# connortannahill/MM-ADMM

Hardware: AMD Instinct MI355X
Metric: ADMM iterations/sec on 1M-node 2D mesh; achieved HBM GB/s in SpMV (higher is better)
Workload: dtype f64

## Files before the change

mm-admm_amd/csrc/host/engine.cpp:

```cpp
#include <algorithm>
#include <chrono>
#include <cmath>
#include <cstring>
#include <limits>
#include <memory>
#include <mutex>
#include <string>
#include <vector>

#include "../../../include/mmx_sparse.h"
#include "../kernels/admm_kernels.h"
#include "../kernels/field_kernels.h"
#include "../kernels/quality_kernels.h"
#include "../kernels/regrid_kernels.h"
#include "../kernels/transfer_kernels.h"
#include "comm.h"
#include "common.h"
#include "partition.h"
#include "transfer.h"
#include "xup_records.h"

#define MMX_SP(expr)                                                                     \
  do {                                                                                   \
    const int rc_ = (expr);                                                              \
// ... 1172 lines not shown
    const CellGrid cg = cellGrid(lo, hi);
    int marg[3] = {0, 0, 0};
    const GridBox R = rowBox(llo, lhi, marg);
    const int passes = smoothPasses();
    const GridBox H = widenBox(R, passes);
    double slo[3] = {0, 0, 0}, shi[3] = {0, 0, 0};
    double diam = 0.0;
    for (int d = 0; d < D; ++d) diam += extMax_[d] * extMax_[d];
    diam = std::sqrt(diam);
    const double marginScale = knobs_.regridMargin;
    for (int d = 0; d < D; ++d) {
      const std::vector<double>& g = d == 0 ? grid_.gx : d == 1 ? grid_.gy : grid_.gz;
      const int sd = (D == 3 && d < 2) ? 1 - d : d;
      const double mu = marginScale * (diam + 2.0 * (g[1] - g[0]));
      slo[d] = g[H.lo[sd]] - mu;
      shi[d] = g[H.hi[sd]] + mu;
    }
    for (int d = 0; d < D; ++d) {
      hs[d] = slo[d];
      hs[D + d] = shi[d];
    }
    smallGather(hs, 2 * D);
    MMX_HIP(hipMemcpyAsync(rgnSbox_.p, hr, sizeof(double) * nranks_ * 2 * D, hipMemcpyHostToDevice, st_));
    MMX_HIP(hipMemsetAsync(rgnCnt_.p, 0, sizeof(int) * (nranks_ + 1), st_));
    launch_select_owned<D>(Vp_.p, ownLocal_.p, rgnOwnGid_.p, nOwned_, nranks_, rank_, rgnSbox_.p, rgnCnt_.p,
                           rgnSend_.p, maxOwned_, st_);
    std::vector<int> cnt(nranks_ + 1);
    MMX_HIP(hipMemcpyAsync(cnt.data(), rgnCnt_.p, sizeof(int) * nranks_, hipMemcpyDeviceToHost, st_));
    streamWait();
    for (int q = 0; q < nranks_; ++q) hs[q] = (double)cnt[q];
    smallGather(hs, nranks_);
    std::vector<HaloPeer> peers;
    int nRecv = 0;
    for (int q = 0; q < nranks_; ++q) {
      if (q == rank_) continue;
      const int sc = cnt[q], rc = (int)hr[(size_t)q * nranks_ + rank_];
      if (sc == 0 && rc == 0) continue;
      HaloPeer p;
      p.rank = q;
      p.sendOff = q * maxOwned_;
      p.sendCount = sc;
      p.recvOff = nRecv;
      p.recvCount = rc;
      nRecv += rc;
      peers.push_back(p);
    }
    const int nCand = nP_ + nRecv;
    if ((int)rgnRecv_.n < std::max(nRecv, 1) * (D + 1)) rgnRecv_.alloc((size_t)std::max(nRecv, 1) * (D + 1) * 2);
    if ((int)rgnCandX_.n < nCand * D) {
      rgnCandX_.alloc((size_t)nCand * D * 2);
      rgnCandGid_.alloc((size_t)nCand * 2);
      rgnCellOf_.alloc((size_t)nCand * 2);
      rgnNodes_.alloc((size_t)nCand * 2);
      rgnMon_.alloc((size_t)nCand * DD * 2);
    }
    comm_->exchange(rank_, rgnSend_.p, rgnRecv_.p, peers, D + 1, st_);
    launch_build_cand<D>(Vp_.p, rgnGid_.p, nP_, rgnRecv_.p, nRecv, rgnCandX_.p, rgnCandGid_.p, st_);
    evalMonitorAt(rgnCandX_.p, nCand, t, rgnMon_.p);
    ensureCells(cg);
    launch_bin<D>(rgnCandX_.p, nCand, cg, rgnCellOf_.p, rgCounts_.p, rgStarts_.p, rgFill_.p, rgnNodes_.p, rgScan_.p,
                  rgScanBytes_, st_);
    double clo[3], chi[3];
    for (int d = 0; d < 3; ++d) {
      clo[d] = (d < D && slo[d] <= lo[d]) ? -INFINITY : slo[d];
      chi[d] = (d < D && shi[d] >= hi[d]) ? INFINITY : shi[d];
    }
    NnCand nc{rgnCandGid_.p, {clo[0], clo[1], clo[2]}, {chi[0], chi[1], chi[2]}, rgnCnt_.p + nranks_};
    launch_nn_fill<D>(rgnCandX_.p, cg, rgStarts_.p, rgnNodes_.p, gx_.p, gy_.p, D == 3 ? gz_.p : gy_.p, grid_.nx,
                      grid_.ny, grid_.nz, rgnMon_.p, rgTmp_.p, H, st_, nc);
    int fail = 0;
    MMX_HIP(hipMemcpyAsync(&fail, rgnCnt_.p + nranks_, sizeof(int), hipMemcpyDeviceToHost, st_));
    streamWait();
    hs[0] = (double)fail;
    smallGather(hs, 1);
    for (int q = 0; q < nranks_; ++q)
      if (hr[q] != 0.0) return false;
    smoothCommit(R, passes, true);
    st_stats_.regrid_rows = (long long)(H.hi[0] - H.lo[0] + 1) * (H.hi[1] - H.lo[1] + 1) * (H.hi[2] - H.lo[2] + 1);
    st_stats_.regrid_gather_bytes = (double)sizeof(double) * ((size_t)nranks_ * (4 * D + nranks_ + 1) +
                                                              (size_t)nRecv * (D + 1));
    st_stats_.regrid_cand = nCand;
    MMX_HIP(hipGetLastError());
    gridOnDevice_ = true;
    updateIso();
    m_ = makeView();
    st_stats_.regrids += 1;
    return true;
  }

  void updateIso() {
    iso_ = false;
    if (!knobs_.iso) return;
    const long long np = (long long)(gvals_.n / (D * D));
    if (np <= 0) return;
    if ((long long)giso_.n != np) giso_.alloc(np);
    if (!isoFlag_.p) isoFlag_.alloc(1);
    MMX_HIP(hipMemsetAsync(isoFlag_.p, 0, sizeof(int), st_));
    launch_iso_compact<D>(gvals_.p, np, giso_.p, isoFlag_.p, st_);
    int notIso = 1;
    MMX_HIP(hipMemcpyAsync(&notIso, isoFlag_.p, sizeof(int), hipMemcpyDeviceToHost, st_));
    streamWait();
    iso_ = (notIso == 0);
  }
  void uploadGridCoords() {
    gx_.upload(grid_.gx.data(), grid_.gx.size(), st_);
    gy_.upload(grid_.gy.data(), grid_.gy.size(), st_);
    if (D == 3) {
      gz_.upload(grid_.gz.data(), grid_.gz.size(), st_);
      const std::vector<double>* ax[3] = {&grid_.gx, &grid_.gy, &grid_.gz};
      for (int a = 0; a < 3; ++a) {
        const std::vector<double>& g = *ax[a];
        const size_t nc = g.size() > 1 ? g.size() - 1 : 1;
        std::vector<double>& t = gcellH_[a];
        t.assign(4 * nc, 0.0);
        for (size_t i = 0; i + 1 < g.size(); ++i) {
          const double h = g[i + 1] - g[i];
          t[4 * i] = g[i];
          t[4 * i + 1] = h;
          t[4 * i + 2] = 1.0 / h;
        }
        gcell_[a].upload(t.data(), t.size(), st_);
      }
    }
  }
  void setGridGeometry(int nG, const double* lo, const double* hi) {
    grid_geometry(D, nG, lo, hi, grid_);
    uploadGridCoords();
  }
  CellGrid cellGrid(const double* lo, const double* hi) const {
    CellGrid cg{};
    const int gn[3] = {grid_.nx, grid_.ny, grid_.nz};
    cg.hmin = INFINITY;
    for (int d = 0; d < 3; ++d) {
      const double ext = d < D ? hi[d] - lo[d] : 0.0;
      cg.lo[d] = d < D ? lo[d] : 0.0;
      cg.n[d] = (d < D && ext > 0) ? std::max(1, gn[d] / 2) : 1;
      cg.inv[d] = (d < D && ext > 0) ? cg.n[d] / ext : 0.0;
      if (d < D && ext > 0) cg.hmin = std::min(cg.hmin, ext / cg.n[d]);
    }
    if (!(cg.hmin < INFINITY)) cg.hmin = 0.0;
    return cg;
  }
  void ensureCells(const CellGrid& cg) {
    const int ncell = cg.n[0] * cg.n[1] * cg.n[2];
    if ((int)rgStarts_.n < ncell + 1) {
      rgCounts_.alloc(ncell + 1);
      rgStarts_.alloc(ncell + 1);
      rgFill_.alloc(ncell);
      rgScanBytes_ = bin_scan_bytes(ncell);
      rgScan_.alloc(std::max<size_t>(rgScanBytes_, 1));
    }
  }
  static int smoothPasses() { return (D == 2) ? 5 : 2; }
  GridBox rowBox(const double* llo, const double* lhi, int* marg) const {
    const int gn3[3] = {grid_.nx, grid_.ny, D == 3 ? grid_.nz : 0};
    GridBox R{{0, 0, 0}, {gn3[0], gn3[1], gn3[2]}};
    for (int d = 0; d < D; ++d) {
      const std::vector<double>& g = d == 0 ? grid_.gx : d == 1 ? grid_.gy : grid_.gz;
      const double h = g[1] - g[0];
      const int M = (int)std::ceil(2.0 * extMax_[d] / h) + 2;
      marg[d] = M;
      R.lo[d] = std::max(0, std::min(gn3[d], (int)std::floor((llo[d] - g[0]) / h) - M));
      R.hi[d] = std::max(0, std::min(gn3[d], (int)std::floor((lhi[d] - g[0]) / h) + 1 + M));
    }
    return R;
  }
  GridBox widenBox(const GridBox& b, int w) const {
    const int gn3[3] = {grid_.nx, grid_.ny, D == 3 ? grid_.nz : 0};
    GridBox o = b;
    for (int d = 0; d < D; ++d) {
      o.lo[d] = std::max(0, b.lo[d] - w);
      o.hi[d] = std::min(gn3[d], b.hi[d] + w);
    }
    return o;
  }
  void evalMonitorAt(const double* X, int n, double t, double* mon) {
    constexpr int DD = D * D;
    if (builtin_monitor_kind(monFn_, monUser_) == 7) {
      double c[3];
      moving_bump_centre(t, c);
      launch_monitor_tv<D>(X, n, c, mon, st_);
    } else {
      std::vector<double> Xh((size_t)n * D), mv((size_t)n * DD);
      MMX_HIP(hipMemcpyAsync(Xh.data(), X, Xh.size() * sizeof(double), hipMemcpyDeviceToHost, st_));
      streamWait();
      for (int v = 0; v < n; ++v) {
        double M[9];
        for (int i = 0; i < DD; ++i) M[i] = 0.0;
        monFn_(D, &Xh[(size_t)v * D], M, monUser_);
        std::memcpy(&mv[(size_t)v * DD], M, DD * sizeof(double));
      }
      MMX_HIP(hipMemcpyAsync(mon, mv.data(), mv.size() * sizeof(double), hipMemcpyHostToDevice, st_));
      streamWait();
    }
  }
  void smoothCommit(const GridBox& R, int passes, bool part) {
    double* cur = rgTmp_.p;
    double* oth = part ? rgTmp2_.p : gvals_.p;
    for (int it = 0; it < passes; ++it) {
      launch_smooth<D>(cur, oth, grid_.nx, grid_.ny, grid_.nz, widenBox(R, part ? passes - 1 - it : 0), st_);
      std::swap(cur, oth);
    }
    if (part) {
      launch_box_commit<D>(cur, gvals_.p, D == 3 ? gpad_.p : nullptr, grid_.nx, grid_.ny, grid_.nz, R, st_);
    } else {
      if (cur != gvals_.p)
        MMX_HIP(hipMemcpyAsync(gvals_.p, cur, gvals_.n * sizeof(double), hipMemcpyDeviceToDevice, st_));
      if (D == 3) launch_pad_rows(gvals_.p, (long long)(gvals_.n / 9), gpad_.p, st_);
    }
  }

  void regridAll(double t, MonSource src = kMonCallback) {
    constexpr int DD = D * D;
    const int nG = (nranks_ > 1) ? plan_.nP : nP_;
    const int nb = std::max(1, std::min(256, (nG + 255) / 256));
    if (!rgPart_.p) {
      rgPart_.alloc((size_t)512 * 2 * D + 256 * D);
      rgMon_.alloc((size_t)nG * DD);
      rgCellOf_.alloc(nG);
      rgNodes_.alloc(nG);
      rgTmp_.alloc(gvals_.n);
      if (nranks_ > 1) rgTmp2_.alloc(gvals_.n);
      if (nranks_ > 1) {
        rgXg_.alloc((size_t)nG * D);
        rgSend_.alloc((size_t)maxOwned_ * D);
        rgRecv_.alloc((size_t)nranks_ * maxOwned_ * D);
      }
      MMX_HIP(hipHostMalloc((void**)&rgHost_, sizeof(double) * (512 * 2 * D + 256 * D), hipHostMallocDefault));
    }
    const double* X = Vp_.p;
    const bool part = nranks_ > 1;
    const int nbl = part ? std::max(1, std::min(256, (nP_ + 255) / 256)) : 0;
    const int nbe = part ? std::max(1, std::min(256, (nF_ + 255) / 256)) : 0;
    double* extPart = rgPart_.p + (size_t)512 * 2 * D;
    if (part) {
      launch_rows_gather(D, ownLocal_.p, nOwned_, Vp_.p, rgSend_.p, st_);
      comm_->allgather(rank_, rgSend_.p, rgRecv_.p, (size_t)maxOwned_ * D, st_);
      launch_rows_scatter(D, ownAllGid_.p, nranks_ * maxOwned_, rgRecv_.p, rgXg_.p, st_);
      X = rgXg_.p;
      launch_bbox<D>(Vp_.p, nP_, rgPart_.p + (size_t)256 * 2 * D, nbl, st_);
      launch_extent<D>(Vp_.p, F_.p, nF_, extPart, nbe, st_);
    }
    launch_bbox<D>(X, nG, rgPart_.p, nb, st_);
    MMX_HIP(hipMemcpyAsync(rgHost_, rgPart_.p, sizeof(double) * nb * 2 * D, hipMemcpyDeviceToHost, st_));
    if (part) {
      MMX_HIP(hipMemcpyAsync(rgHost_ + (size_t)256 * 2 * D, rgPart_.p + (size_t)256 * 2 * D, sizeof(double) * nbl * 2 * D,
                             hipMemcpyDeviceToHost, st_));
      MMX_HIP(hipMemcpyAsync(rgHost_ + (size_t)512 * 2 * D, extPart, sizeof(double) * nbe * D, hipMemcpyDeviceToHost,
                             st_));
    }
    streamWait();
    double lo[3] = {INFINITY, INFINITY, INFINITY}, hi[3] = {-INFINITY, -INFINITY, -INFINITY};
    double llo[3] = {INFINITY, INFINITY, INFINITY}, lhi[3] = {-INFINITY, -INFINITY, -INFINITY};
    for (int b = 0; b < nb; ++b)
      for (int d = 0; d < D; ++d) {
        lo[d] = std::min(lo[d], rgHost_[(size_t)b * 2 * D + d]);
        hi[d] = std::max(hi[d], rgHost_[(size_t)b * 2 * D + D + d]);
      }
    for (int b = 0; b < nbl; ++b)
      for (int d = 0; d < D; ++d) {
        llo[d] = std::min(llo[d], rgHost_[(size_t)(256 + b) * 2 * D + d]);
        lhi[d] = std::max(lhi[d], rgHost_[(size_t)(256 + b) * 2 * D + D + d]);
      }
    if (part) {
      for (int d = 0; d < D; ++d) extMax_[d] = 0.0;
      for (int b = 0; b < nbe; ++b)
        for (int d = 0; d < D; ++d) extMax_[d] = std::max(extMax_[d], rgHost_[(size_t)512 * 2 * D + (size_t)b * D + d]);
    }
    grid_geometry(D, nG, lo, hi, grid_);
    uploadGridCoords();
    CellGrid cg{};
    const int gn[3] = {grid_.nx, grid_.ny, grid_.nz};
    cg.hmin = INFINITY;
    for (int d = 0; d < 3; ++d) {
      const double ext = d < D ? hi[d] - lo[d] : 0.0;
      cg.lo[d] = d < D ? lo[d] : 0.0;
      cg.n[d] = (d < D && ext > 0) ? std::max(1, gn[d] / 2) : 1;
      cg.inv[d] = (d < D && ext > 0) ? cg.n[d] / ext : 0.0;
      if (d < D && ext > 0) cg.hmin = std::min(cg.hmin, ext / cg.n[d]);
    }
    if (!(cg.hmin < INFINITY)) cg.hmin = 0.0;
    const int ncell = cg.n[0] * cg.n[1] * cg.n[2];
    if ((int)rgStarts_.n < ncell + 1) {
      rgCounts_.alloc(ncell + 1);
      rgStarts_.alloc(ncell + 1);
      rgFill_.alloc(ncell);
      rgScanBytes_ = bin_scan_bytes(ncell);
      rgScan_.alloc(std::max<size_t>(rgScanBytes_, 1));
    }
    launch_bin<D>(X, nG, cg, rgCellOf_.p, rgCounts_.p, rgStarts_.p, rgFill_.p, rgNodes_.p, rgScan_.p, rgScanBytes_,
                  st_);
    if (src == kMonCallback && builtin_monitor_kind(monFn_, monUser_) == 7) src = kMonBuiltin7;
    if (src == kMonValues) {
      MMX_HIP(hipMemcpyAsync(rgMon_.p, srcPtr_, (size_t)nG * DD * sizeof(double), hipMemcpyDeviceToDevice, st_));
    } else if (src == kMonField) {
      fieldScratch();
      launch_field_hessian<D>(X, srcPtr_, F_.p, nF_, incPtr_.p, incOff_.p, nodeOrder_.p, nP_, fldE_.p, fldG_.p,
                              srcAlpha_, nullptr, rgMon_.p, st_);
    } else if (src == kMonFieldHuang) {
      fieldHuangMonitor(X);
    } else if (src == kMonBuiltin7) {
      double c[3];
      moving_bump_centre(t, c);
      launch_monitor_tv<D>(X, nG, c, rgMon_.p, st_);
    } else {
      std::vector<double> Xh((size_t)nG * D), mv((size_t)nG * DD);
      MMX_HIP(hipMemcpyAsync(Xh.data(), X, Xh.size() * sizeof(double), hipMemcpyDeviceToHost, st_));
      streamWait();
      for (int v = 0; v < nG; ++v) {
        double M[9];
        for (int i = 0; i < DD; ++i) M[i] = 0.0;
        monFn_(D, &Xh[(size_t)v * D], M, monUser_);
        std::memcpy(&mv[(size_t)v * DD], M, DD * sizeof(double));
      }
      MMX_HIP(hipMemcpyAsync(rgMon_.p, mv.data(), mv.size() * sizeof(double), hipMemcpyHostToDevice, st_));
      streamWait();
    }
    const int passes = (D == 2) ? 5 : 2;
    const int gn3[3] = {grid_.nx, grid_.ny, D == 3 ? grid_.nz : 0};
    GridBox R{{0, 0, 0}, {gn3[0], gn3[1], gn3[2]}};
    if (part) {
      for (int d = 0; d < D; ++d) {
        const std::vector<double>& g = d == 0 ? grid_.gx : d == 1 ? grid_.gy : grid_.gz;
        const double h = g[1] - g[0];
        const int M = (int)std::ceil(2.0 * extMax_[d] / h) + 2;
        R.lo[d] = std::max(0, std::min(gn3[d], (int)std::floor((llo[d] - g[0]) / h) - M));
        R.hi[d] = std::max(0, std::min(gn3[d], (int)std::floor((lhi[d] - g[0]) / h) + 1 + M));
      }
    }
    auto widen = [&](const GridBox& b, int w) {
      GridBox o = b;
      for (int d = 0; d < D; ++d) {
        o.lo[d] = std::max(0, b.lo[d] - w);
        o.hi[d] = std::min(gn3[d], b.hi[d] + w);
      }
      return o;
    };
    const GridBox H = widen(R, part ? passes : 0);
    launch_nn_fill<D>(X, cg, rgStarts_.p, rgNodes_.p, gx_.p, gy_.p, D == 3 ? gz_.p : gy_.p, grid_.nx, grid_.ny,
                      grid_.nz, rgMon_.p, rgTmp_.p, H, st_);
    double* cur = rgTmp_.p;
    double* oth = part ? rgTmp2_.p : gvals_.p;
    for (int it = 0; it < passes; ++it) {
      launch_smooth<D>(cur, oth, grid_.nx, grid_.ny, grid_.nz, widen(R, part ? passes - 1 - it : 0), st_);
      std::swap(cur, oth);
    }
    if (part) {
      launch_box_commit<D>(cur, gvals_.p, D == 3 ? gpad_.p : nullptr, grid_.nx, grid_.ny, grid_.nz, R, st_);
    } else {
      if (cur != gvals_.p)
        MMX_HIP(hipMemcpyAsync(gvals_.p, cur, gvals_.n * sizeof(double), hipMemcpyDeviceToDevice, st_));
      if (D == 3) launch_pad_rows(gvals_.p, (long long)(gvals_.n / 9), gpad_.p, st_);
    }
    st_stats_.regrid_rows = (long long)(H.hi[0] - H.lo[0] + 1) * (H.hi[1] - H.lo[1] + 1) * (H.hi[2] - H.lo[2] + 1);
    st_stats_.regrid_gather_bytes = part ? (double)nranks_ * maxOwned_ * D * sizeof(double) : 0.0;
    st_stats_.regrid_cand = part ? nG : 0;
    MMX_HIP(hipGetLastError());
    gridOnDevice_ = true;
    updateIso();
    m_ = makeView();
    st_stats_.regrids += 1;
  }

  DeviceMesh<D> makeView() const {
    DeviceMesh<D> m{};
    m.nP = nP_;
    m.nF = nF_;
    m.F = F_.p;
    m.sbits = sbits_.p;
    m.nodeInterior = interior_.p;
    m.inc_ptr = incPtr_.p;
    m.inc_off = incOff_.p;
    m.remote = nranks_ > 1 ? remote_.p : nullptr;
    m.tslot = knobs_.tslot ? tslot_.p : nullptr;
    m.gcache = gcache_.p;
    m.tieList = tieList_.p;
    m.tieCount = tieCount_.p + tiePar_;
    m.tieStale = tieCount_.p + (tiePar_ ^ 1);
    m.invFlag = tieCount_.p + 2;
    m.nodeOrder = nodeOrder_.p;
    m.xupLo = 0;
    m.xupHi = nP_;
    m.prox2dWave = knobs_.prox2dWave;
    m.xupSweep = knobs_.xupSweep;
    m.xupCh = knobs_.xupCh;
    m.xupEarly = knobs_.xupEarly;
    m.forceTie = knobs_.forceTie;
    m.monHint = knobs_.monHint;
    if (knobs_.xupRec) {
      m.xrec = xrec_.p;
      m.xinv = xinv_.p;
      m.xslot = xslot_.p;
      m.xslotStride = xslotStride_;
      m.xslotCh = xslotCh_;
    }
    m.invdiag = invdiag_.p;
    m.Vc = compMesh_ ? Vc_.p : nullptr;
    m.gx = gx_.p;
    m.gy = gy_.p;
    m.gz = (D == 3) ? gz_.p : gy_.p;
    m.gvals = gvals_.p;
    m.gpad = (D == 3) ? gpad_.p : nullptr;
    for (int a = 0; a < 3; ++a) m.gcell[a] = (D == 3) ? gcell_[a].p : nullptr;
    m.giso = iso_ ? giso_.p : nullptr;
    m.gnx = grid_.nx;
    m.gny = grid_.ny;
    m.gnz = grid_.nz;
    m.ghx = grid_.gx[1] - grid_.gx[0];
    m.ghy = grid_.gy[1] - grid_.gy[0];
    m.ghz = (D == 3) ? grid_.gz[1] - grid_.gz[0] : 1.0;
    m.grhx = 1.0 / m.ghx;
    m.grhy = 1.0 / m.ghy;
    m.grhz = 1.0 / m.ghz;
    const int ns[3] = {grid_.nx, grid_.ny, grid_.nz};
    double* A[3] = {&m.gax, &m.gay, &m.gaz};
    double* SP[3] = {&m.gspx, &m.gspy, &m.gspz};
    double* NS[3] = {&m.gnsx, &m.gnsy, &m.gnsz};
    double* RNS[3] = {&m.grnsx, &m.grnsy, &m.grnsz};
    for (int d = 0; d < 3; ++d) {
      const bool on = d < D;
      *A[d] = on ? grid_.lo[d] : 0.0;
      *SP[d] = on ? grid_.hi[d] - grid_.lo[d] : 0.0;
      *NS[d] = on ? (double)ns[d] : 1.0;
      *RNS[d] = 1.0 / *NS[d];
    }
    for (int i = 0; i < D * D; ++i) m.Ehat[i] = EhatH_[i];
    m.powd = powd_;
    m.w = w_;
    m.compMesh = compMesh_ ? 1 : 0;
    return m;
  }

  void ensureResults(int nIters) {
    if (nIters <= resultsCap_) return;
    resultsCap_ = std::max(nIters, 64);
    const size_t n = (size_t)resultsCap_ * 2 * kNumPartials;
    if (nranks_ == 1 && knobs_.spin) {
      if (resH_) MMX_HIP(hipHostFree(resH_));
      resH_ = nullptr;
      MMX_HIP(hipHostMalloc((void**)&resH_, n * sizeof(double), hipHostMallocMapped));
      MMX_HIP(hipHostGetDevicePointer((void**)&res_, resH_, 0));
    } else {
// ... 452 lines not shown
```

mm-admm_amd/csrc/kernels/regrid_kernels.h:

```cpp
#pragma once
#include <hip/hip_runtime.h>
#include <stddef.h>

namespace mmx {

struct CellGrid {
  double lo[3];
  double inv[3];
  int n[3];
  double hmin;
};

struct GridBox {
  int lo[3];
  int hi[3];
};

template <int D>
void launch_bbox(const double* X, int n, double* partials, int nblocks, hipStream_t st);
template <int D>
void launch_extent(const double* X, const int* F, int nF, double* partials, int nblocks, hipStream_t st);
template <int D>
void launch_bin(const double* X, int n, const CellGrid& cg, int* cellOfV, int* counts, int* starts, int* fill,
                int* cellNodes, void* scanTmp, size_t scanTmpBytes, hipStream_t st);
size_t bin_scan_bytes(int ncell);
template <int D>
void launch_monitor_tv(const double* X, int n, const double* c, double* monVals, hipStream_t st);
struct NnCand {
  const int* gid;
  double slo[3], shi[3];
  int* fail;
};
template <int D>
void launch_nn_fill(const double* X, const CellGrid& cg, const int* starts, const int* cellNodes, const double* gx,
                    const double* gy, const double* gz, int nx, int ny, int nz, const double* monVals, double* vals,
                    const GridBox& box, hipStream_t st, const NnCand& cand = NnCand{nullptr, {0, 0, 0}, {0, 0, 0}, nullptr});
template <int D>
void launch_select_owned(const double* X, const int* ownLocal, const int* ownGid, int nOwned, int nranks, int rank,
                         const double* sboxes, int* counts, double* send, int cap, hipStream_t st);
template <int D>
void launch_build_cand(const double* X, const int* gidLocal, int nLocal, const double* recv, int nRecv, double* cx,
                       int* cgid, hipStream_t st);
template <int D>
void launch_smooth(const double* in, double* out, int nx, int ny, int nz, const GridBox& box, hipStream_t st);
template <int D>
void launch_box_commit(const double* src, double* vals, double* pad, int nx, int ny, int nz, const GridBox& box,
                       hipStream_t st);

void launch_rows_gather(int D, const int* idx, int n, const double* in, double* out, hipStream_t st);
void launch_rows_scatter(int D, const int* idx, int n, const double* in, double* out, hipStream_t st);

}
```

mm-admm_amd/csrc/kernels/regrid_kernels.hip:

```cpp
#include <hip/hip_runtime.h>

#include <hipcub/hipcub.hpp>

#include "regrid_kernels.h"

namespace mmx {
namespace {

constexpr int kRB = 256;

template <int D>
__global__ void __launch_bounds__(kRB) k_bbox(const double* __restrict__ X, int n, double* __restrict__ part) {
  __shared__ double sm[2 * D][kRB];
  double lo[D], hi[D];
#pragma unroll
  for (int d = 0; d < D; ++d) {
    lo[d] = INFINITY;
    hi[d] = -INFINITY;
  }
  for (int v = blockIdx.x * kRB + threadIdx.x; v < n; v += gridDim.x * kRB)
#pragma unroll
    for (int d = 0; d < D; ++d) {
      const double x = X[(size_t)v * D + d];
      lo[d] = x < lo[d] ? x : lo[d];
// ... 30 lines not shown
#pragma unroll
    for (int n = 0; n <= D; ++n) v[n] = F[(size_t)s * (D + 1) + n];
#pragma unroll
    for (int d = 0; d < D; ++d) {
      double a = X[(size_t)v[0] * D + d], b = a;
#pragma unroll
      for (int n = 1; n <= D; ++n) {
        const double c = X[(size_t)v[n] * D + d];
        a = c < a ? c : a;
        b = c > b ? c : b;
      }
      const double e = b - a;
      ext[d] = e > ext[d] ? e : ext[d];
    }
  }
#pragma unroll
  for (int d = 0; d < D; ++d) sm[d][threadIdx.x] = ext[d];
  __syncthreads();
  for (int w = kRB / 2; w > 0; w >>= 1) {
    if ((int)threadIdx.x < w)
#pragma unroll
      for (int d = 0; d < D; ++d) {
        const double a = sm[d][threadIdx.x + w];
        sm[d][threadIdx.x] = a > sm[d][threadIdx.x] ? a : sm[d][threadIdx.x];
      }
    __syncthreads();
  }
  if (threadIdx.x < D) part[(size_t)blockIdx.x * D + threadIdx.x] = sm[threadIdx.x][0];
}

template <int D>
__device__ __forceinline__ int cellOf(const double* x, const CellGrid& cg, int (&c)[3]) {
  int id = 0;
#pragma unroll
  for (int d = D - 1; d >= 0; --d) {
    int k = (int)((x[d] - cg.lo[d]) * cg.inv[d]);
    k = k < 0 ? 0 : (k >= cg.n[d] ? cg.n[d] - 1 : k);
    c[d] = k;
    id = id * cg.n[d] + k;
  }
  return id;
}

template <int D>
__global__ void __launch_bounds__(kRB) k_bin_count(const double* __restrict__ X, int n, CellGrid cg,
                                                   int* __restrict__ cellOfV, int* __restrict__ counts) {
  const int v = blockIdx.x * kRB + threadIdx.x;
  if (v >= n) return;
  double x[D];
#pragma unroll
  for (int d = 0; d < D; ++d) x[d] = X[(size_t)v * D + d];
  int c[3];
  const int id = cellOf<D>(x, cg, c);
  cellOfV[v] = id;
  atomicAdd(&counts[id], 1);
}

__global__ void __launch_bounds__(kRB) k_bin_fill(int n, const int* __restrict__ cellOfV,
                                                  const int* __restrict__ starts, int* __restrict__ fill,
                                                  int* __restrict__ cellNodes) {
  const int v = blockIdx.x * kRB + threadIdx.x;
  if (v >= n) return;
  const int c = cellOfV[v];
  cellNodes[starts[c] + atomicAdd(&fill[c], 1)] = v;
}

template <int D>
__global__ void __launch_bounds__(kRB) k_monitor_tv(const double* __restrict__ X, int n, double c0, double c1,
                                                    double c2, double* __restrict__ monVals) {
  const int v = blockIdx.x * kRB + threadIdx.x;
  if (v >= n) return;
  const double c[3] = {c0, c1, c2};
  double sq = 0.0;
#pragma unroll
  for (int d = 0; d < D; ++d) {
    const double t = X[(size_t)v * D + d] - c[d];
    sq = (d == 0) ? t * t : sq + t * t;
  }
  const double s = 1 + 5.0 / (1 + 50.0 * sq);
#pragma unroll
  for (int i = 0; i < D * D; ++i) monVals[(size_t)v * D * D + i] = (i / D == i % D) ? s : 0.0;
}

__device__ __forceinline__ size_t box_row(const GridBox& b, long long p, int nx, int ny, int& sx, int& sy, int& sk) {
  const long long bx = b.hi[0] - b.lo[0] + 1, by = b.hi[1] - b.lo[1] + 1;
  sx = b.lo[0] + (int)(p % bx);
  sy = b.lo[1] + (int)((p / bx) % by);
  sk = b.lo[2] + (int)(p / (bx * by));
  return ((size_t)sk * (ny + 1) + sy) * (nx + 1) + sx;
}
__device__ __forceinline__ long long box_rows(const GridBox& b) {
  return (long long)(b.hi[0] - b.lo[0] + 1) * (b.hi[1] - b.lo[1] + 1) * (b.hi[2] - b.lo[2] + 1);
}

template <int D>
__global__ void __launch_bounds__(kRB) k_nn_fill(const double* __restrict__ X, CellGrid cg,
                                                 const int* __restrict__ starts, const int* __restrict__ cellNodes,
                                                 const double* __restrict__ gx, const double* __restrict__ gy,
                                                 const double* __restrict__ gz, int nx, int ny, int nz,
                                                 const double* __restrict__ monVals, double* __restrict__ vals,
                                                 GridBox box, NnCand cand) {
  constexpr int DD = D * D;
  const long long p = (long long)blockIdx.x * kRB + threadIdx.x;
  if (p >= box_rows(box)) return;
  int sx, sy, k;
  const size_t row = box_row(box, p, nx, ny, sx, sy, k);
  const int i = (D == 2) ? sx : sy, j = (D == 2) ? sy : sx;
  double q[3] = {gx[i], gy[j], D == 3 ? gz[k] : 0.0};
  int c[3] = {0, 0, 0};
  cellOf<D>(q, cg, c);
  double best = INFINITY;
  int bi = -1, bg = -1;
  int rmax = 0;
#pragma unroll
  for (int d = 0; d < D; ++d) rmax = max(rmax, max(c[d], cg.n[d] - 1 - c[d]));
  for (int r = 0; r <= rmax; ++r) {
    const int z0 = (D == 3) ? max(c[2] - r, 0) : 0, z1 = (D == 3) ? min(c[2] + r, cg.n[2] - 1) : 0;
    const int y0 = max(c[1] - r, 0), y1 = min(c[1] + r, cg.n[1] - 1);
    const int x0 = max(c[0] - r, 0), x1 = min(c[0] + r, cg.n[0] - 1);
    for (int cz = z0; cz <= z1; ++cz)
      for (int cy = y0; cy <= y1; ++cy)
        for (int cx = x0; cx <= x1; ++cx) {
          const int dz = (D == 3) ? abs(cz - c[2]) : 0;
          if (max(max(abs(cx - c[0]), abs(cy - c[1])), dz) != r) continue;
          const int cell = (cz * cg.n[1] + cy) * cg.n[0] + cx;
          for (int t = starts[cell]; t < starts[cell + 1]; ++t) {
            const int v = cellNodes[t];
            const int gv = cand.gid ? cand.gid[v] : v;
            double dd = 0.0;
#pragma unroll
            for (int d = 0; d < D; ++d) {
              const double df = q[d] - X[(size_t)v * D + d];
              dd += df * df;
            }
            if (dd < best || (dd == best && gv < bg)) {
              best = dd;
              bi = v;
              bg = gv;
            }
          }
        }
    const double lb = ((double)r - 1e-6) * cg.hmin;
    if (bi >= 0 && r > 0 && best < lb * lb) break;
  }
  if (cand.gid) {
    double gap = INFINITY;
#pragma unroll
    for (int d = 0; d < D; ++d) gap = fmin(gap, fmin(q[d] - cand.slo[d], cand.shi[d] - q[d]));
    if (!(bi >= 0 && gap > 0.0 && best < gap * gap * (1.0 - 1e-9))) {
      atomicOr(cand.fail, 1);
      if (bi < 0) return;
    }
  }
#pragma unroll
  for (int e = 0; e < DD; ++e) vals[row * DD + e] = monVals[(size_t)bi * DD + e];
}

template <int D>
__global__ void __launch_bounds__(kRB) k_select_owned(const double* __restrict__ X, const int* __restrict__ ownLocal,
                                                      const int* __restrict__ ownGid, int nOwned, int nranks, int rank,
                                                      const double* __restrict__ sboxes, int* __restrict__ counts,
                                                      double* __restrict__ send, int cap) {
  const int i = blockIdx.x * kRB + threadIdx.x;
  if (i >= nOwned) return;
  const int v = ownLocal[i];
  double x[D];
#pragma unroll
  for (int d = 0; d < D; ++d) x[d] = X[(size_t)v * D + d];
  for (int q = 0; q < nranks; ++q) {
    if (q == rank) continue;
    const double* s = sboxes + (size_t)q * 2 * D;
    bool in = true;
#pragma unroll
    for (int d = 0; d < D; ++d) in = in && x[d] >= s[d] && x[d] <= s[D + d];
    if (in) {
      const int k = atomicAdd(&counts[q], 1);
      double* r = send + ((size_t)q * cap + k) * (D + 1);
#pragma unroll
      for (int d = 0; d < D; ++d) r[d] = x[d];
      r[D] = (double)ownGid[i];
    }
  }
}

template <int D>
__global__ void __launch_bounds__(kRB) k_build_cand(const double* __restrict__ X, const int* __restrict__ gidLocal,
                                                    int nLocal, const double* __restrict__ recv, int nRecv,
                                                    double* __restrict__ cx, int* __restrict__ cgid) {
  const int i = blockIdx.x * kRB + threadIdx.x;
  if (i >= nLocal + nRecv) return;
  if (i < nLocal) {
#pragma unroll
    for (int d = 0; d < D; ++d) cx[(size_t)i * D + d] = X[(size_t)i * D + d];
    cgid[i] = gidLocal[i];
  } else {
    const double* r = recv + (size_t)(i - nLocal) * (D + 1);
#pragma unroll
    for (int d = 0; d < D; ++d) cx[(size_t)i * D + d] = r[d];
    cgid[i] = (int)r[D];
  }
}

template <int D>
__global__ void __launch_bounds__(kRB) k_smooth(const double* __restrict__ in, double* __restrict__ out, int nx,
                                                int ny, int nz, GridBox box) {
  constexpr int DD = D * D;
  const long long p = (long long)blockIdx.x * kRB + threadIdx.x;
  const long long P = (long long)(nx + 1) * (ny + 1);
  if (p >= box_rows(box)) return;
  int i, j, k;
  const long long c = (long long)box_row(box, p, nx, ny, i, j, k);
  const bool interior = i >= 1 && i < nx && j >= 1 && j < ny && (D == 2 || (k >= 1 && k < nz));
  for (int q = 0; q < DD; ++q) {
    double v;
    if (!interior) {
      v = in[c * DD + q];
    } else if constexpr (D == 2) {
      v = 0.6 * in[c * DD + q];
      v += 0.1 * in[(c + 1) * DD + q];
      v += 0.1 * in[(c - 1) * DD + q];
      v += 0.1 * in[(c + nx + 1) * DD + q];
      v += 0.1 * in[(c - nx - 1) * DD + q];
    } else {
      const double h = 0.4 / 6.0;
      v = 0.6 * in[c * DD + q] + h * in[(c + 1) * DD + q] + h * in[(c - 1) * DD + q] + h * in[(c + nx + 1) * DD + q] +
          h * in[(c - nx - 1) * DD + q] + h * in[(c + P) * DD + q] + h * in[(c - P) * DD + q];
    }
    out[c * DD + q] = v;
  }
}

template <int D>
__global__ void __launch_bounds__(kRB) k_box_commit(const double* __restrict__ src, double* __restrict__ vals,
                                                    double* __restrict__ pad, int nx, int ny, int nz, GridBox box) {
  constexpr int DD = D * D;
  const long long c = (long long)blockIdx.x * kRB + threadIdx.x;
  const long long P = (long long)(nx + 1) * (ny + 1);
  if (c >= P * (D == 3 ? nz + 1 : 1)) return;
  const int i = (int)(c % (nx + 1)), j = (int)((c / (nx + 1)) % (ny + 1)), k = (D == 3) ? (int)(c / P) : 0;
  const bool in = i >= box.lo[0] && i <= box.hi[0] && j >= box.lo[1] && j <= box.hi[1] && k >= box.lo[2] &&
                  k <= box.hi[2];
  const double nan = __builtin_nan("");
  for (int q = 0; q < DD; ++q) vals[c * DD + q] = in ? src[c * DD + q] : nan;
  if (D == 3 && pad) {
    for (int q = 0; q < DD; ++q) pad[c * 10 + q] = in ? src[c * DD + q] : nan;
    pad[c * 10 + 9] = 0.0;
  }
}

__global__ void __launch_bounds__(kRB) k_rows_gather(int D, const int* __restrict__ idx, int n,
                                                     const double* __restrict__ in, double* __restrict__ out) {
  const int i = blockIdx.x * kRB + threadIdx.x;
  if (i >= n) return;
  for (int c = 0; c < D; ++c) out[(size_t)i * D + c] = in[(size_t)idx[i] * D + c];
}
__global__ void __launch_bounds__(kRB) k_rows_scatter(int D, const int* __restrict__ idx, int n,
                                                      const double* __restrict__ in, double* __restrict__ out) {
  const int i = blockIdx.x * kRB + threadIdx.x;
  if (i >= n || idx[i] < 0) return;
  for (int c = 0; c < D; ++c) out[(size_t)idx[i] * D + c] = in[(size_t)i * D + c];
}

inline unsigned blocks(long long n) { return (unsigned)((n + kRB - 1) / kRB); }

}

template <int D>
void launch_bbox(const double* X, int n, double* partials, int nblocks, hipStream_t st) {
  hipLaunchKernelGGL(k_bbox<D>, dim3(nblocks), dim3(kRB), 0, st, X, n, partials);
}

template <int D>
void launch_extent(const double* X, const int* F, int nF, double* partials, int nblocks, hipStream_t st) {
  hipLaunchKernelGGL(k_extent<D>, dim3(nblocks), dim3(kRB), 0, st, X, F, nF, partials);
}

template <int D>
void launch_bin(const double* X, int n, const CellGrid& cg, int* cellOfV, int* counts, int* starts, int* fill,
                int* cellNodes, void* scanTmp, size_t scanTmpBytes, hipStream_t st) {
  const int ncell = cg.n[0] * cg.n[1] * cg.n[2];
  (void)hipMemsetAsync(counts, 0, sizeof(int) * (ncell + 1), st);
  (void)hipMemsetAsync(fill, 0, sizeof(int) * ncell, st);
  hipLaunchKernelGGL(k_bin_count<D>, dim3(blocks(n)), dim3(kRB), 0, st, X, n, cg, cellOfV, counts);
  size_t bytes = scanTmpBytes;
  (void)hipcub::DeviceScan::ExclusiveSum(scanTmp, bytes, counts, starts, ncell + 1, st);
  hipLaunchKernelGGL(k_bin_fill, dim3(blocks(n)), dim3(kRB), 0, st, n, cellOfV, starts, fill, cellNodes);
}

size_t bin_scan_bytes(int ncell) {
  size_t bytes = 0;
  (void)hipcub::DeviceScan::ExclusiveSum(nullptr, bytes, (int*)nullptr, (int*)nullptr, ncell + 1, (hipStream_t)0);
  return bytes;
}

template <int D>
void launch_monitor_tv(const double* X, int n, const double* c, double* monVals, hipStream_t st) {
  hipLaunchKernelGGL(k_monitor_tv<D>, dim3(blocks(n)), dim3(kRB), 0, st, X, n, c[0], c[1], c[2], monVals);
}

static long long host_box_rows(const GridBox& b) {
  return (long long)(b.hi[0] - b.lo[0] + 1) * (b.hi[1] - b.lo[1] + 1) * (b.hi[2] - b.lo[2] + 1);
}

template <int D>
void launch_nn_fill(const double* X, const CellGrid& cg, const int* starts, const int* cellNodes, const double* gx,
                    const double* gy, const double* gz, int nx, int ny, int nz, const double* monVals, double* vals,
                    const GridBox& box, hipStream_t st, const NnCand& cand) {
  const long long n = host_box_rows(box);
  if (n > 0)
    hipLaunchKernelGGL(k_nn_fill<D>, dim3(blocks(n)), dim3(kRB), 0, st, X, cg, starts, cellNodes, gx, gy, gz, nx, ny,
                       nz, monVals, vals, box, cand);
}

template <int D>
void launch_select_owned(const double* X, const int* ownLocal, const int* ownGid, int nOwned, int nranks, int rank,
                         const double* sboxes, int* counts, double* send, int cap, hipStream_t st) {
  if (nOwned > 0)
    hipLaunchKernelGGL(k_select_owned<D>, dim3(blocks(nOwned)), dim3(kRB), 0, st, X, ownLocal, ownGid, nOwned, nranks,
                       rank, sboxes, counts, send, cap);
}

template <int D>
void launch_build_cand(const double* X, const int* gidLocal, int nLocal, const double* recv, int nRecv, double* cx,
                       int* cgid, hipStream_t st) {
  if (nLocal + nRecv > 0)
    hipLaunchKernelGGL(k_build_cand<D>, dim3(blocks(nLocal + nRecv)), dim3(kRB), 0, st, X, gidLocal, nLocal, recv,
                       nRecv, cx, cgid);
}

template <int D>
void launch_smooth(const double* in, double* out, int nx, int ny, int nz, const GridBox& box, hipStream_t st) {
  const long long n = host_box_rows(box);
  if (n > 0) hipLaunchKernelGGL(k_smooth<D>, dim3(blocks(n)), dim3(kRB), 0, st, in, out, nx, ny, nz, box);
}

template <int D>
void launch_box_commit(const double* src, double* vals, double* pad, int nx, int ny, int nz, const GridBox& box,
                       hipStream_t st) {
  const long long rows = (long long)(nx + 1) * (ny + 1) * (D == 3 ? nz + 1 : 1);
  hipLaunchKernelGGL(k_box_commit<D>, dim3(blocks(rows)), dim3(kRB), 0, st, src, vals, pad, nx, ny, nz, box);
}

void launch_rows_gather(int D, const int* idx, int n, const double* in, double* out, hipStream_t st) {
  if (n > 0) hipLaunchKernelGGL(k_rows_gather, dim3(blocks(n)), dim3(kRB), 0, st, D, idx, n, in, out);
}
void launch_rows_scatter(int D, const int* idx, int n, const double* in, double* out, hipStream_t st) {
  if (n > 0) hipLaunchKernelGGL(k_rows_scatter, dim3(blocks(n)), dim3(kRB), 0, st, D, idx, n, in, out);
}

#define MMX_REGRID_INST(D)                                                                                       \
  template void launch_bbox<D>(const double*, int, double*, int, hipStream_t);                                 \
  template void launch_extent<D>(const double*, const int*, int, double*, int, hipStream_t);                    \
  template void launch_bin<D>(const double*, int, const CellGrid&, int*, int*, int*, int*, int*, void*, size_t, \
                              hipStream_t);                                                                    \
  template void launch_monitor_tv<D>(const double*, int, const double*, double*, hipStream_t);                  \
  template void launch_nn_fill<D>(const double*, const CellGrid&, const int*, const int*, const double*,        \
                                  const double*, const double*, int, int, int, const double*, double*,          \
                                  const GridBox&, hipStream_t, const NnCand&);                                 \
  template void launch_select_owned<D>(const double*, const int*, const int*, int, int, int, const double*, int*, \
                                       double*, int, hipStream_t);                                               \
  template void launch_build_cand<D>(const double*, const int*, int, const double*, int, double*, int*,          \
                                     hipStream_t);                                                               \
  template void launch_smooth<D>(const double*, double*, int, int, int, const GridBox&, hipStream_t);           \
  template void launch_box_commit<D>(const double*, double*, double*, int, int, int, const GridBox&, hipStream_t);
MMX_REGRID_INST(2)
MMX_REGRID_INST(3)
#undef MMX_REGRID_INST

}
```

Measured before the change: 2617.

## Fuse iso/pad derivation into final smooth pass and coalesce regrid writes

```diff
diff --git a/mm-admm_amd/csrc/host/engine.cpp b/mm-admm_amd/csrc/host/engine.cpp
--- a/mm-admm_amd/csrc/host/engine.cpp
+++ b/mm-admm_amd/csrc/host/engine.cpp
@@ -1278,25 +1278,33 @@
     st_stats_.regrid_cand = nCand;
     MMX_HIP(hipGetLastError());
     gridOnDevice_ = true;
-    updateIso();
+    updateIso(true);
     m_ = makeView();
     st_stats_.regrids += 1;
     return true;
   }
 
-  void updateIso() {
+  void updateIso(bool written = false) {
     iso_ = false;
-    if (!knobs_.iso) return;
-    const long long np = (long long)(gvals_.n / (D * D));
-    if (np <= 0) return;
-    if ((long long)giso_.n != np) giso_.alloc(np);
-    if (!isoFlag_.p) isoFlag_.alloc(1);
-    MMX_HIP(hipMemsetAsync(isoFlag_.p, 0, sizeof(int), st_));
-    launch_iso_compact<D>(gvals_.p, np, giso_.p, isoFlag_.p, st_);
+    if (!written) {
+      if (!isoBuffers()) return;
+      launch_iso_compact<D>(gvals_.p, (long long)giso_.n, giso_.p, isoFlag_.p, st_);
+    } else if (!knobs_.iso || !giso_.p) {
+      return;
+    }
     int notIso = 1;
     MMX_HIP(hipMemcpyAsync(&notIso, isoFlag_.p, sizeof(int), hipMemcpyDeviceToHost, st_));
     streamWait();
     iso_ = (notIso == 0);
+  }
+  bool isoBuffers() {
+    if (!knobs_.iso) return false;
+    const long long np = (long long)(gvals_.n / (D * D));
+    if (np <= 0) return false;
+    if ((long long)giso_.n != np) giso_.alloc(np);
+    if (!isoFlag_.p) isoFlag_.alloc(1);
+    MMX_HIP(hipMemsetAsync(isoFlag_.p, 0, sizeof(int), st_));
+    return true;
   }
   void uploadGridCoords() {
     gx_.upload(grid_.gx.data(), grid_.gx.size(), st_);
@@ -1391,20 +1399,21 @@
     }
   }
   void smoothCommit(const GridBox& R, int passes, bool part) {
-    double* cur = rgTmp_.p;
-    double* oth = part ? rgTmp2_.p : gvals_.p;
+    GridDerived der{D == 3 ? gpad_.p : nullptr, nullptr, nullptr};
+    if (isoBuffers()) {
+      der.iso = giso_.p;
+      der.notIso = isoFlag_.p;
+    }
+    double* cur = fillTarget(passes, part);
+    double* oth = part ? rgTmp2_.p : (cur == gvals_.p ? rgTmp_.p : gvals_.p);
     for (int it = 0; it < passes; ++it) {
-      launch_smooth<D>(cur, oth, grid_.nx, grid_.ny, grid_.nz, widenBox(R, part ? passes - 1 - it : 0), st_);
+      launch_smooth<D>(cur, oth, grid_.nx, grid_.ny, grid_.nz, widenBox(R, part ? passes - 1 - it : 0), st_,
+                       (!part && it == passes - 1) ? &der : nullptr);
       std::swap(cur, oth);
     }
-    if (part) {
-      launch_box_commit<D>(cur, gvals_.p, D == 3 ? gpad_.p : nullptr, grid_.nx, grid_.ny, grid_.nz, R, st_);
-    } else {
-      if (cur != gvals_.p)
-        MMX_HIP(hipMemcpyAsync(gvals_.p, cur, gvals_.n * sizeof(double), hipMemcpyDeviceToDevice, st_));
-      if (D == 3) launch_pad_rows(gvals_.p, (long long)(gvals_.n / 9), gpad_.p, st_);
-    }
-  }
+    if (part) launch_box_commit<D>(cur, gvals_.p, grid_.nx, grid_.ny, grid_.nz, R, der, st_);
+  }
+  double* fillTarget(int passes, bool part) const { return (part || passes % 2) ? rgTmp_.p : gvals_.p; }
 
   void regridAll(double t, MonSource src = kMonCallback) {
     constexpr int DD = D * D;
@@ -1534,26 +1543,14 @@
     };
     const GridBox H = widen(R, part ? passes : 0);
     launch_nn_fill<D>(X, cg, rgStarts_.p, rgNodes_.p, gx_.p, gy_.p, D == 3 ? gz_.p : gy_.p, grid_.nx, grid_.ny,
-                      grid_.nz, rgMon_.p, rgTmp_.p, H, st_);
-    double* cur = rgTmp_.p;
-    double* oth = part ? rgTmp2_.p : gvals_.p;
-    for (int it = 0; it < passes; ++it) {
-      launch_smooth<D>(cur, oth, grid_.nx, grid_.ny, grid_.nz, widen(R, part ? passes - 1 - it : 0), st_);
-      std::swap(cur, oth);
-    }
-    if (part) {
-      launch_box_commit<D>(cur, gvals_.p, D == 3 ? gpad_.p : nullptr, grid_.nx, grid_.ny, grid_.nz, R, st_);
-    } else {
-      if (cur != gvals_.p)
-        MMX_HIP(hipMemcpyAsync(gvals_.p, cur, gvals_.n * sizeof(double), hipMemcpyDeviceToDevice, st_));
-      if (D == 3) launch_pad_rows(gvals_.p, (long long)(gvals_.n / 9), gpad_.p, st_);
-    }
+                      grid_.nz, rgMon_.p, fillTarget(passes, part), H, st_);
+    smoothCommit(R, passes, part);
     st_stats_.regrid_rows = (long long)(H.hi[0] - H.lo[0] + 1) * (H.hi[1] - H.lo[1] + 1) * (H.hi[2] - H.lo[2] + 1);
     st_stats_.regrid_gather_bytes = part ? (double)nranks_ * maxOwned_ * D * sizeof(double) : 0.0;
     st_stats_.regrid_cand = part ? nG : 0;
     MMX_HIP(hipGetLastError());
     gridOnDevice_ = true;
-    updateIso();
+    updateIso(true);
     m_ = makeView();
     st_stats_.regrids += 1;
   }
diff --git a/mm-admm_amd/csrc/kernels/regrid_kernels.h b/mm-admm_amd/csrc/kernels/regrid_kernels.h
--- a/mm-admm_amd/csrc/kernels/regrid_kernels.h
+++ b/mm-admm_amd/csrc/kernels/regrid_kernels.h
@@ -1,6 +1,8 @@
 #pragma once
 #include <hip/hip_runtime.h>
 #include <stddef.h>
+
+#include "regrid_map.h"
 
 namespace mmx {
 
@@ -9,11 +11,6 @@
   double inv[3];
   int n[3];
   double hmin;
-};
-
-struct GridBox {
-  int lo[3];
-  int hi[3];
 };
 
 template <int D>
@@ -41,11 +38,17 @@
 template <int D>
 void launch_build_cand(const double* X, const int* gidLocal, int nLocal, const double* recv, int nRecv, double* cx,
                        int* cgid, hipStream_t st);
+struct GridDerived {
+  double* pad;
+  double* iso;
+  int* notIso;
+};
 template <int D>
-void launch_smooth(const double* in, double* out, int nx, int ny, int nz, const GridBox& box, hipStream_t st);
+void launch_smooth(const double* in, double* out, int nx, int ny, int nz, const GridBox& box, hipStream_t st,
+                   const GridDerived* last = nullptr);
 template <int D>
-void launch_box_commit(const double* src, double* vals, double* pad, int nx, int ny, int nz, const GridBox& box,
-                       hipStream_t st);
+void launch_box_commit(const double* src, double* vals, int nx, int ny, int nz, const GridBox& box,
+                       const GridDerived& der, hipStream_t st);
 
 void launch_rows_gather(int D, const int* idx, int n, const double* in, double* out, hipStream_t st);
 void launch_rows_scatter(int D, const int* idx, int n, const double* in, double* out, hipStream_t st);
diff --git a/mm-admm_amd/csrc/kernels/regrid_kernels.hip b/mm-admm_amd/csrc/kernels/regrid_kernels.hip
--- a/mm-admm_amd/csrc/kernels/regrid_kernels.hip
+++ b/mm-admm_amd/csrc/kernels/regrid_kernels.hip
@@ -136,29 +136,16 @@
   for (int i = 0; i < D * D; ++i) monVals[(size_t)v * D * D + i] = (i / D == i % D) ? s : 0.0;
 }
 
-__device__ __forceinline__ size_t box_row(const GridBox& b, long long p, int nx, int ny, int& sx, int& sy, int& sk) {
-  const long long bx = b.hi[0] - b.lo[0] + 1, by = b.hi[1] - b.lo[1] + 1;
-  sx = b.lo[0] + (int)(p % bx);
-  sy = b.lo[1] + (int)((p / bx) % by);
-  sk = b.lo[2] + (int)(p / (bx * by));
-  return ((size_t)sk * (ny + 1) + sy) * (nx + 1) + sx;
-}
-__device__ __forceinline__ long long box_rows(const GridBox& b) {
-  return (long long)(b.hi[0] - b.lo[0] + 1) * (b.hi[1] - b.lo[1] + 1) * (b.hi[2] - b.lo[2] + 1);
-}
-
-template <int D>
-__global__ void __launch_bounds__(kRB) k_nn_fill(const double* __restrict__ X, CellGrid cg,
-                                                 const int* __restrict__ starts, const int* __restrict__ cellNodes,
-                                                 const double* __restrict__ gx, const double* __restrict__ gy,
-                                                 const double* __restrict__ gz, int nx, int ny, int nz,
-                                                 const double* __restrict__ monVals, double* __restrict__ vals,
-                                                 GridBox box, NnCand cand) {
-  constexpr int DD = D * D;
-  const long long p = (long long)blockIdx.x * kRB + threadIdx.x;
-  if (p >= box_rows(box)) return;
+static_assert(kRB == kRegridWG, "regrid_map.h's workgroup maps are for this block size");
+
+template <int D>
+__device__ __forceinline__ int nn_search(const double* __restrict__ X, const CellGrid& cg,
+                                         const int* __restrict__ starts, const int* __restrict__ cellNodes,
+                                         const double* __restrict__ gx, const double* __restrict__ gy,
+                                         const double* __restrict__ gz, int nx, int ny, const GridBox& box,
+                                         const NnCand& cand, long long p, long long& row) {
   int sx, sy, k;
-  const size_t row = box_row(box, p, nx, ny, sx, sy, k);
+  row = box_row(box, p, nx, ny, sx, sy, k);
   const int i = (D == 2) ? sx : sy, j = (D == 2) ? sy : sx;
   double q[3] = {gx[i], gy[j], D == 3 ? gz[k] : 0.0};
   int c[3] = {0, 0, 0};
@@ -201,13 +188,42 @@
     double gap = INFINITY;
 #pragma unroll
     for (int d = 0; d < D; ++d) gap = fmin(gap, fmin(q[d] - cand.slo[d], cand.shi[d] - q[d]));
-    if (!(bi >= 0 && gap > 0.0 && best < gap * gap * (1.0 - 1e-9))) {
-      atomicOr(cand.fail, 1);
-      if (bi < 0) return;
-    }
-  }
-#pragma unroll
-  for (int e = 0; e < DD; ++e) vals[row * DD + e] = monVals[(size_t)bi * DD + e];
+    if (!(bi >= 0 && gap > 0.0 && best < gap * gap * (1.0 - 1e-9))) atomicOr(cand.fail, 1);
+  }
+  return bi;
+}
+
+template <int D>
+__global__ void __launch_bounds__(kRB) k_nn_fill(const double* __restrict__ X, CellGrid cg,
+                                                 const int* __restrict__ starts, const int* __restrict__ cellNodes,
+                                                 const double* __restrict__ gx, const double* __restrict__ gy,
+                                                 const double* __restrict__ gz, int nx, int ny, int nz,
+                                                 const double* __restrict__ monVals, double* __restrict__ vals,
+                                                 GridBox box, NnCand cand) {
+  constexpr int DD = D * D;
+  const long long p0 = (long long)blockIdx.x * kRB, nrows = box_rows(box);
+  int bi = -1;
+  long long row = 0;
+  if (p0 + threadIdx.x < nrows)
+    bi = nn_search<D>(X, cg, starts, cellNodes, gx, gy, gz, nx, ny, box, cand, p0 + threadIdx.x, row);
+#ifdef MMX_NNFILL_DIRECT
+  if (bi >= 0)
+#pragma unroll
+    for (int e = 0; e < DD; ++e) vals[row * DD + e] = monVals[(size_t)bi * DD + e];
+#else
+  __shared__ long long srow[kRB];
+  __shared__ int sbi[kRB];
+  srow[threadIdx.x] = row;
+  sbi[threadIdx.x] = bi;
+  __syncthreads();
+  const int nrow = (int)(nrows - p0 < kRB ? nrows - p0 : kRB);
+  for (int t = threadIdx.x; t < nrow * DD; t += kRB) {
+    int pl, e;
+    wg_entry<D>(t, pl, e);
+    const int v = sbi[pl];
+    if (v >= 0) vals[srow[pl] * DD + e] = monVals[(size_t)v * DD + e];
+  }
+#endif
 }
 
 template <int D>
@@ -256,50 +272,100 @@
 }
 
 template <int D>
+__device__ __forceinline__ void grid_derived(const double* sval, const long long* srow, int nrow,
+                                             const GridDerived& der) {
+  constexpr int DD = D * D;
+  if (der.iso && (int)threadIdx.x < nrow) {
+    const double* v = sval + threadIdx.x * DD;
+    const unsigned long long d0 = __double_as_longlong(v[0]);
+    bool ok = true, nan = true;
+#pragma unroll
+    for (int k = 0; k < DD; ++k) {
+      const unsigned long long b = __double_as_longlong(v[k]);
+      ok = ok && (b == ((k / D == k % D) ? d0 : 0ull));
+      nan = nan && (v[k] != v[k]);
+    }
+    if (!(ok || nan)) *der.notIso = 1;
+    der.iso[srow[threadIdx.x]] = v[0];
+  }
+  if (D == 3 && der.pad)
+    for (int t = threadIdx.x; t < nrow * 10; t += kRB) {
+      const int pl = t / 10, n = t - pl * 10;
+      der.pad[srow[pl] * 10 + n] = (n < 9) ? sval[pl * 9 + n] : 0.0;
+    }
+}
+
+template <int D, bool LAST>
 __global__ void __launch_bounds__(kRB) k_smooth(const double* __restrict__ in, double* __restrict__ out, int nx,
-                                                int ny, int nz, GridBox box) {
+                                                int ny, int nz, GridBox box, GridDerived der) {
   constexpr int DD = D * D;
-  const long long p = (long long)blockIdx.x * kRB + threadIdx.x;
-  const long long P = (long long)(nx + 1) * (ny + 1);
-  if (p >= box_rows(box)) return;
-  int i, j, k;
-  const long long c = (long long)box_row(box, p, nx, ny, i, j, k);
-  const bool interior = i >= 1 && i < nx && j >= 1 && j < ny && (D == 2 || (k >= 1 && k < nz));
-  for (int q = 0; q < DD; ++q) {
+  __shared__ long long srow[kRB];
+  __shared__ int sint[kRB];
+  __shared__ double sval[LAST ? kRB * DD : 1];
+  const long long p0 = (long long)blockIdx.x * kRB, nrows = box_rows(box);
+  const int nrow = (int)(nrows - p0 < kRB ? nrows - p0 : kRB);
+  if ((int)threadIdx.x < nrow) {
+    int i, j, k;
+    srow[threadIdx.x] = box_row(box, p0 + threadIdx.x, nx, ny, i, j, k);
+    sint[threadIdx.x] = grid_interior<D>(i, j, k, nx, ny, nz);
+  }
+  __syncthreads();
+  const long long sy = (long long)(nx + 1) * DD, sz = sy * (ny + 1);
+  for (int t = threadIdx.x; t < nrow * DD; t += kRB) {
+    int pl, q;
+    wg_entry<D>(t, pl, q);
+    const long long e = srow[pl] * DD + q;
+    const double* a = in + e;
     double v;
-    if (!interior) {
-      v = in[c * DD + q];
+    if (!sint[pl]) {
+      v = a[0];
     } else if constexpr (D == 2) {
-      v = 0.6 * in[c * DD + q];
-      v += 0.1 * in[(c + 1) * DD + q];
-      v += 0.1 * in[(c - 1) * DD + q];
-      v += 0.1 * in[(c + nx + 1) * DD + q];
-      v += 0.1 * in[(c - nx - 1) * DD + q];
+      v = 0.6 * a[0];
+      v += 0.1 * a[DD];
+      v += 0.1 * a[-DD];
+      v += 0.1 * a[sy];
+      v += 0.1 * a[-sy];
     } else {
       const double h = 0.4 / 6.0;
-      v = 0.6 * in[c * DD + q] + h * in[(c + 1) * DD + q] + h * in[(c - 1) * DD + q] + h * in[(c + nx + 1) * DD + q] +
-          h * in[(c - nx - 1) * DD + q] + h * in[(c + P) * DD + q] + h * in[(c - P) * DD + q];
-    }
-    out[c * DD + q] = v;
-  }
-}
-
-template <int D>
-__global__ void __launch_bounds__(kRB) k_box_commit(const double* __restrict__ src, double* __restrict__ vals,
-                                                    double* __restrict__ pad, int nx, int ny, int nz, GridBox box) {
+      v = 0.6 * a[0] + h * a[DD] + h * a[-DD] + h * a[sy] + h * a[-sy] + h * a[sz] + h * a[-sz];
+    }
+    out[e] = v;
+    if constexpr (LAST) sval[t] = v;
+  }
+  if constexpr (LAST) {
+    __syncthreads();
+    grid_derived<D>(sval, srow, nrow, der);
+  }
+}
+
+template <int D>
+__global__ void __launch_bounds__(kRB) k_box_commit(const double* __restrict__ src, double* __restrict__ vals, int nx,
+                                                    int ny, int nz, GridBox box, GridDerived der) {
   constexpr int DD = D * D;
-  const long long c = (long long)blockIdx.x * kRB + threadIdx.x;
-  const long long P = (long long)(nx + 1) * (ny + 1);
-  if (c >= P * (D == 3 ? nz + 1 : 1)) return;
-  const int i = (int)(c % (nx + 1)), j = (int)((c / (nx + 1)) % (ny + 1)), k = (D == 3) ? (int)(c / P) : 0;
-  const bool in = i >= box.lo[0] && i <= box.hi[0] && j >= box.lo[1] && j <= box.hi[1] && k >= box.lo[2] &&
-                  k <= box.hi[2];
+  __shared__ long long srow[kRB];
+  __shared__ int sin[kRB];
+  __shared__ double sval[kRB * DD];
+  const GridBox full{{0, 0, 0}, {nx, ny, D == 3 ? nz : 0}};
+  const long long p0 = (long long)blockIdx.x * kRB, nrows = box_rows(full);
+  const int nrow = (int)(nrows - p0 < kRB ? nrows - p0 : kRB);
+  if ((int)threadIdx.x < nrow) {
+    int i, j, k;
+    srow[threadIdx.x] = box_row(full, p0 + threadIdx.x, nx, ny, i, j, k);
+    sin[threadIdx.x] = i >= box.lo[0] && i <= box.hi[0] && j >= box.lo[1] && j <= box.hi[1] && k >= box.lo[2] &&
+                       k <= box.hi[2];
+  }
+  __syncthreads();
   const double nan = __builtin_nan("");
-  for (int q = 0; q < DD; ++q) vals[c * DD + q] = in ? src[c * DD + q] : nan;
-  if (D == 3 && pad) {
-    for (int q = 0; q < DD; ++q) pad[c * 10 + q] = in ? src[c * DD + q] : nan;
-    pad[c * 10 + 9] = 0.0;
-  }
+  for (int t = threadIdx.x; t < nrow * DD; t += kRB) {
+    int pl, q;
+    wg_entry<D>(t, pl, q);
+    const long long e = srow[pl] * DD + q;
+    const double v = sin[pl] ? src[e] : nan;
+    vals[e] = v;
+    sval[t] = v;
+  }
+  __syncthreads();
+  grid_derived<D>(sval, srow, nrow, der);
 }
 
 __global__ void __launch_bounds__(kRB) k_rows_gather(int D, const int* __restrict__ idx, int n,
@@ -352,15 +418,11 @@
   hipLaunchKernelGGL(k_monitor_tv<D>, dim3(blocks(n)), dim3(kRB), 0, st, X, n, c[0], c[1], c[2], monVals);
 }
 
-static long long host_box_rows(const GridBox& b) {
-  return (long long)(b.hi[0] - b.lo[0] + 1) * (b.hi[1] - b.lo[1] + 1) * (b.hi[2] - b.lo[2] + 1);
-}
-
 template <int D>
 void launch_nn_fill(const double* X, const CellGrid& cg, const int* starts, const int* cellNodes, const double* gx,
                     const double* gy, const double* gz, int nx, int ny, int nz, const double* monVals, double* vals,
                     const GridBox& box, hipStream_t st, const NnCand& cand) {
-  const long long n = host_box_rows(box);
+  const long long n = box_rows(box);
   if (n > 0)
     hipLaunchKernelGGL(k_nn_fill<D>, dim3(blocks(n)), dim3(kRB), 0, st, X, cg, starts, cellNodes, gx, gy, gz, nx, ny,
                        nz, monVals, vals, box, cand);
@@ -383,16 +445,22 @@
 }
 
 template <int D>
-void launch_smooth(const double* in, double* out, int nx, int ny, int nz, const GridBox& box, hipStream_t st) {
-  const long long n = host_box_rows(box);
-  if (n > 0) hipLaunchKernelGGL(k_smooth<D>, dim3(blocks(n)), dim3(kRB), 0, st, in, out, nx, ny, nz, box);
-}
-
-template <int D>
-void launch_box_commit(const double* src, double* vals, double* pad, int nx, int ny, int nz, const GridBox& box,
-                       hipStream_t st) {
+void launch_smooth(const double* in, double* out, int nx, int ny, int nz, const GridBox& box, hipStream_t st,
+                   const GridDerived* last) {
+  const long long n = box_rows(box);
+  if (n <= 0) return;
+  if (last)
+    hipLaunchKernelGGL((k_smooth<D, true>), dim3(blocks(n)), dim3(kRB), 0, st, in, out, nx, ny, nz, box, *last);
+  else
+    hipLaunchKernelGGL((k_smooth<D, false>), dim3(blocks(n)), dim3(kRB), 0, st, in, out, nx, ny, nz, box,
+                       GridDerived{nullptr, nullptr, nullptr});
+}
+
+template <int D>
+void launch_box_commit(const double* src, double* vals, int nx, int ny, int nz, const GridBox& box,
+                       const GridDerived& der, hipStream_t st) {
   const long long rows = (long long)(nx + 1) * (ny + 1) * (D == 3 ? nz + 1 : 1);
-  hipLaunchKernelGGL(k_box_commit<D>, dim3(blocks(rows)), dim3(kRB), 0, st, src, vals, pad, nx, ny, nz, box);
+  hipLaunchKernelGGL(k_box_commit<D>, dim3(blocks(rows)), dim3(kRB), 0, st, src, vals, nx, ny, nz, box, der);
 }
 
 void launch_rows_gather(int D, const int* idx, int n, const double* in, double* out, hipStream_t st) {
@@ -415,8 +483,10 @@
                                        double*, int, hipStream_t);                                               \
   template void launch_build_cand<D>(const double*, const int*, int, const double*, int, double*, int*,          \
                                      hipStream_t);                                                               \
-  template void launch_smooth<D>(const double*, double*, int, int, int, const GridBox&, hipStream_t);           \
-  template void launch_box_commit<D>(const double*, double*, double*, int, int, int, const GridBox&, hipStream_t);
+  template void launch_smooth<D>(const double*, double*, int, int, int, const GridBox&, hipStream_t,           \
+                                 const GridDerived*);                                                            \
+  template void launch_box_commit<D>(const double*, double*, int, int, int, const GridBox&, const GridDerived&, \
+                                     hipStream_t);
 MMX_REGRID_INST(2)
 MMX_REGRID_INST(3)
 #undef MMX_REGRID_INST
diff --git a/mm-admm_amd/csrc/kernels/regrid_map.h b/mm-admm_amd/csrc/kernels/regrid_map.h
--- /dev/null
+++ b/mm-admm_amd/csrc/kernels/regrid_map.h
@@ -0,0 +1,71 @@
+#pragma once
+
+#if defined(__HIPCC__)
+#define MMX_MAP_HD __host__ __device__ __forceinline__
+#else
+#define MMX_MAP_HD inline
+#endif
+
+namespace mmx {
+
+struct GridBox {
+  int lo[3];
+  int hi[3];
+};
+
+constexpr int kRegridWG = 256;
+
+MMX_MAP_HD long long box_rows(const GridBox& b) {
+  return (long long)(b.hi[0] - b.lo[0] + 1) * (b.hi[1] - b.lo[1] + 1) * (b.hi[2] - b.lo[2] + 1);
+}
+
+MMX_MAP_HD long long box_row(const GridBox& b, long long p, int nx, int ny, int& sx, int& sy, int& sk) {
+  const long long bx = b.hi[0] - b.lo[0] + 1, by = b.hi[1] - b.lo[1] + 1;
+  if (p <= 0xffffffffll) {
+    const unsigned pu = (unsigned)p, bxu = (unsigned)bx, byu = (unsigned)by;
+    const unsigned ru = pu / bxu;
+    sx = b.lo[0] + (int)(pu - ru * bxu);
+    const unsigned tu = ru / byu;
+    sy = b.lo[1] + (int)(ru - tu * byu);
+    sk = b.lo[2] + (int)tu;
+  } else {
+    const long long r = p / bx;
+    sx = b.lo[0] + (int)(p - r * bx);
+    const long long t = r / by;
+    sy = b.lo[1] + (int)(r - t * by);
+    sk = b.lo[2] + (int)t;
+  }
+  return ((long long)sk * (ny + 1) + sy) * (nx + 1) + sx;
+}
+
+template <int D>
+MMX_MAP_HD bool grid_interior(int i, int j, int k, int nx, int ny, int nz) {
+  return i >= 1 && i < nx && j >= 1 && j < ny && (D == 2 || (k >= 1 && k < nz));
+}
+
+template <int D>
+MMX_MAP_HD void wg_entry(int t, int& pl, int& q) {
+  pl = t / (D * D);
+  q = t - pl * (D * D);
+}
+
+struct GridEntry {
+  long long row;
+  int q;
+  int i, j, k;
+  bool interior;
+};
+template <int D>
+MMX_MAP_HD GridEntry grid_entry(const GridBox& b, long long e, int nx, int ny, int nz) {
+  constexpr long long W = (long long)kRegridWG * D * D;
+  const long long wg = e / W;
+  int pl, q;
+  wg_entry<D>((int)(e - wg * W), pl, q);
+  GridEntry g;
+  g.q = q;
+  g.row = box_row(b, wg * kRegridWG + pl, nx, ny, g.i, g.j, g.k);
+  g.interior = grid_interior<D>(g.i, g.j, g.k, nx, ny, nz);
+  return g;
+}
+
+}
```

New measurement: 2609. Within noise of the previous version (-0.3%).
